# KleistLab/ADAPTed

Measured on AMD Instinct MI355X. Metric: reads/sec (adapter+polyA detect), RNA004 200k-sample reads, higher is better.
Workload: dtype f32 samples/statistics, f64 cumulative sums + LLR trace

## Files before the change

adapted_amd/csrc/adapted_hip.hip:

```cpp
#include <hip/hip_runtime.h>

#include <cmath>
#include <cstdio>
#include <cstring>
#include <cstdlib>
#include <string>
#include <vector>

#include "adapted_hip.h"
#include "handle.h"
#include "common.h"
__device__ unsigned long long g_dbg[ADP_NDBG] = {0};
__device__ unsigned long long g_bs_tally[ADP_NTALLY][8] = {{0}};
#include "llr_stream.h"
#include "n1_select.h"
#include "n1_fused.h"
#include "peaks.h"
#include "synth.h"
#include "validate.h"
#include "cand_stats2.h"
#include "series_pipe.h"
#include "cnn_topk.h"
#include "cnn_conv.h"
#include "cnn_conv_split.h"
// ... 449 lines not shown
                     const int32_t *tails = nullptr)
{
    hipStream_t st = h->stream;
    h->n1_fused_nmb = 0;
    MbState *mbs = h->mbs.as<MbState>();
    uint32_t *gh = h->ghist.as<uint32_t>(), *gb = h->gbelow.as<uint32_t>();
    unsigned long long *gc = h->gcnt.as<unsigned long long>();
    const int collect = ((long long)minibatch * T >= (1ll << 24)) ? 1 : 0;
    ALLOCCHK(collect && h->cbuf.ensure((size_t)n_mb * N1_CB_CAP * 4));
    uint32_t *cb = h->cbuf.as<uint32_t>();
    int bpm = 4096 / n_mb; if (bpm > 256) bpm = 256; if (bpm < 4) bpm = 4;
    dim3 hg(bpm, n_mb), pg(n_mb);
    const int pdiv = 32;
    int col_div = 1;
    if (T >= 8192) { col_div = T / (pdiv * 96); if (col_div > 64) col_div = 64; if (col_div < 2) col_div = 2; }
    int row_step = (col_div > 1) ? 1 : minibatch / 32; if (row_step < 1) row_step = 1;
    int sb = (minibatch + row_step - 1) / row_step; if (sb > bpm) sb = bpm; if (sb < 1) sb = 1;
    dim3 sg(sb, n_mb);
    const double thr = h->cfg.sig_norm_outlier_thresh;
    const long long fused_min = getenv("ADP_N1_FUSED_MIN") ? atoll(getenv("ADP_N1_FUSED_MIN")) : (1ll << 22);
    if ((long long)minibatch * T >= fused_min && T >= 64) {
        ALLOCCHK(h->cbuf.ensure((size_t)n_mb * N1_CB_CAP * 4) || h->fz.ensure((size_t)n_mb * sizeof(N1Fused)) ||
                 h->fcnt.ensure((size_t)n_mb * 8 * N1F_NCNT) || h->n1heavy.ensure((size_t)n_mb * N1H_WORDS * 4));
        cb = h->cbuf.as<uint32_t>();
        h->n1_fused_nmb = n_mb;
        N1Fused *fz = h->fz.as<N1Fused>();
        unsigned long long *fc = h->fcnt.as<unsigned long long>();
        HIPCHK(hipMemsetAsync(fc, 0, (size_t)n_mb * 8 * N1F_NCNT, st));
        uint32_t *hvy = h->n1heavy.as<uint32_t>();
        HIPCHK(hipMemsetAsync(hvy, 0, (size_t)n_mb * N1H_WORDS * 4, st));
        { Scope s(h, !profile ? nullptr : "k_n1 sample passes");
        const int s0 = (col_div > 1 && minibatch >= 64) ? env_int("ADP_N1_S0", 8) : 1;
        for (int mode = 0; mode < 2; mode++) {
            hipLaunchKernelGGL((k_n1_hist<0, SIG>), sg, dim3(N1_THREADS), 0, st, dsig, n, m, T, minibatch, mode, mbs, gh, gb, gc, row_step * (s0 > 1 ? s0 : 1), N1_ALWAYS, cb, 0, col_div, pdiv, tails);
            hipLaunchKernelGGL((k_n1_pick<0, N1_SAMPLE>), pg, dim3(256), 0, st, mbs, gh, gb, gc, mode, thr);
            hipLaunchKernelGGL((k_n1_hist<1, SIG>), sg, dim3(N1_THREADS), 0, st, dsig, n, m, T, minibatch, mode, mbs, gh, gb, gc, row_step, N1_ALWAYS, cb, 0, col_div, pdiv, tails);
            hipLaunchKernelGGL((k_n1_pick<1, N1_SAMPLE>), pg, dim3(256), 0, st, mbs, gh, gb, gc, mode, thr);
            hipLaunchKernelGGL(k_n1_fuse_setup, dim3((n_mb + 63) / 64), dim3(64), 0, st, mbs, fz, n_mb, mode);
        }
        hipLaunchKernelGGL(k_n1_heavy_scan<SIG>, dim3((sb + 3) / 4, n_mb), dim3(N1_THREADS), 0, st, dsig, n, m, T, minibatch, mbs, fz, hvy, row_step * 4, col_div, pdiv, tails);
        hipLaunchKernelGGL(k_n1_heavy_pick, pg, dim3(64), 0, st, mbs, fz, hvy, n_mb); }
        { Scope s(h, !profile ? nullptr : "k_n1_fused");
          hipLaunchKernelGGL(k_n1_fused<SIG>, hg, dim3(N1_THREADS), 0, st, dsig, n, m, T, minibatch, mbs, fz, fc, (float *)cb, hvy, tails); }
        { Scope s(h, !profile ? nullptr : "k_n1_fused_finish");
          hipLaunchKernelGGL(k_n1_fused_finish, pg, dim3(1024), 0, st, mbs, fz, fc, (const float *)cb, thr, (const uint32_t *)hvy); }
    }
    if ((long long)minibatch * T >= fused_min && T >= 64 && bpm < 128) hg = dim3(128, n_mb);
    for (int mode = 0; mode < 2; mode++) {
        hipLaunchKernelGGL((k_n1_hist<0, SIG>), sg, dim3(N1_THREADS), 0, st, dsig, n, m, T, minibatch, mode, mbs, gh, gb, gc, row_step, N1_ALWAYS, cb, 0, col_div, pdiv, tails);
        hipLaunchKernelGGL((k_n1_pick<0, N1_SAMPLE>), pg, dim3(256), 0, st, mbs, gh, gb, gc, mode, thr);
        hipLaunchKernelGGL((k_n1_hist<1, SIG>), sg, dim3(N1_THREADS), 0, st, dsig, n, m, T, minibatch, mode, mbs, gh, gb, gc, row_step, N1_ALWAYS, cb, 0, col_div, pdiv, tails);
        hipLaunchKernelGGL((k_n1_pick<1, N1_SAMPLE>), pg, dim3(256), 0, st, mbs, gh, gb, gc, mode, thr);
        { Scope s(h, !profile ? nullptr : (mode ? "k_n1_hist<1> mad" : "k_n1_hist<1> med"));
          hipLaunchKernelGGL((k_n1_hist<1, SIG>), hg, dim3(N1_THREADS), 0, st, dsig, n, m, T, minibatch, mode, mbs, gh, gb, gc, 1, N1_ALWAYS, cb, collect, 1, 8, tails); }
        hipLaunchKernelGGL((k_n1_pick<1, N1_FULL>), pg, dim3(256), 0, st, mbs, gh, gb, gc, mode, thr);
        hipLaunchKernelGGL(k_n1_finish, pg, dim3(1024), 0, st, mbs, cb, gc, gb, mode, thr);
        hipLaunchKernelGGL((k_n1_hist<0, SIG>), hg, dim3(N1_THREADS), 0, st, dsig, n, m, T, minibatch, mode, mbs, gh, gb, gc, 1, N1_IF_BAD, cb, 0, 1, 8, tails);
        hipLaunchKernelGGL((k_n1_pick<0, N1_FALLBACK>), pg, dim3(256), 0, st, mbs, gh, gb, gc, mode, thr);
        hipLaunchKernelGGL((k_n1_hist<1, SIG>), hg, dim3(N1_THREADS), 0, st, dsig, n, m, T, minibatch, mode, mbs, gh, gb, gc, 1, N1_IF_BAD, cb, 0, 1, 8, tails);
        hipLaunchKernelGGL((k_n1_pick<1, N1_FALLBACK>), pg, dim3(256), 0, st, mbs, gh, gb, gc, mode, thr);
        { Scope s(h, !profile ? nullptr : (mode ? "k_n1_hist<2> mad" : "k_n1_hist<2> med"));
          hipLaunchKernelGGL((k_n1_hist<2, SIG>), hg, dim3(N1_THREADS), 0, st, dsig, n, m, T, minibatch, mode, mbs, gh, gb, gc, 1, N1_IF_NOT_DONE, cb, 0, 1, 8, tails); }
        hipLaunchKernelGGL((k_n1_pick<2, N1_FULL>), pg, dim3(256), 0, st, mbs, gh, gb, gc, mode, thr);
    }
    return 0;
}

struct PhaseSync {
    hipEvent_t wait[3] = {nullptr, nullptr, nullptr};
    hipEvent_t done[3] = {nullptr, nullptr, nullptr};
};

static __device__ __host__ inline SigF32 sig_from(const SigF32 &s, size_t r0, int m) { return SigF32{s.base + r0 * (size_t)m}; }
static __device__ __host__ inline SigI16 sig_from(const SigI16 &s, size_t r0, int m) { return SigI16{s.base + r0 * (size_t)m, s.scale + r0, s.offset + r0, s.full_len + r0}; }
static inline SigIdx sig_subset(const SigF32 &s, const int32_t *sel) { return SigIdx{s.base, sel}; }
static inline SigIdxI16 sig_subset(const SigI16 &s, const int32_t *sel) { return SigIdxI16{s.base, s.scale, s.offset, s.full_len, sel}; }

static void launch_cumsum(adp_handle *h, int n)
{
    const int split = env_int("ADP_CUMSUM_GATHER", 1) != 0;
    hipLaunchKernelGGL(k_cumsum, dim3((n + 63) / 64), dim3(64), 0, h->stream, h->down.as<float>(), h->nvalid.as<int32_t>(), h->Lp, n,
                       h->nck, h->ck.as<double2>(), h->tail.as<double2>(), split);
    if (split)
        hipLaunchKernelGGL(k_cumsum_gather, dim3((n + 63) / 64), dim3(64), 0, h->stream, h->down.as<float>(), h->nvalid.as<int32_t>(), h->Lp, n,
                           h->nck, h->ck.as<double2>(), h->tail.as<double2>());
}

static int gains_tile_fast() { return env_int("ADP_GAINS_TILE_FAST", 1) != 0; }

#define G2_WINDOW_DEFAULT 1024
static int g2_window(int upto)
{
    const char *e = getenv("ADP_G2_WINDOW");
    if (!e || !*e) return upto >= 8 ? G2_WINDOW_DEFAULT : 0;
    const int w = env_int("ADP_G2_WINDOW", G2_WINDOW_DEFAULT);
    return w < 0 ? 0 : (w > (1 << 28) ? (1 << 28) : w);
}
static void launch_gains2(adp_handle *h, int n, int mbsize, double *pkv, int win, const int32_t *redo, const MbState *mbs = nullptr)
{
    hipLaunchKernelGGL(k_gains<2>, dim3((n + GAINS_WPB - 1) / GAINS_WPB), dim3(64 * GAINS_WPB), 0, h->stream, h->down.as<float>(), h->nvalid.as<int32_t>(), h->Lp, h->nck,
                       h->ck.as<double2>(), h->tail.as<double2>(), h->adapter_idx.as<int32_t>(), mbsize, mbs ? mbs : h->mbs.as<MbState>(),
                       h->trace.as<double>(), h->bmax.as<double>(), h->bmin.as<double>(), h->nsum, h->t1.as<int2>(), 0, h->pk.as<int32_t>(), h->npk.as<int32_t>(), h->Lp / 2 + 1, h->gstat.as<double>(), n, 5, pkv, gains_tile_fast(),
                       win, h->wend.as<int32_t>(), redo);
}

static void launch_polya_peak(adp_handle *h, int n, int mbsize, const double *pkv, bool windowed = false, bool redo_pass = false, const MbState *mbs = nullptr)
{
    const int grid = n < h->pslots ? n : h->pslots;
    hipLaunchKernelGGL(k_polya_peak, dim3(grid), dim3(64), (size_t)(((h->Lp / 2 + 1) + 8) / 16 + 2) * 4, h->stream, h->trace.as<double>(), h->nvalid.as<int32_t>(), h->Lp,
                       h->bmax.as<double>(), h->bmin.as<double>(), h->nsum, h->adapter_idx.as<int32_t>(), n, mbsize, mbs ? mbs : h->mbs.as<MbState>(),
                       h->pk.as<int32_t>(), h->mk.as<uint32_t>(), h->polya_idx.as<int32_t>(), h->npk.as<int32_t>(), pkv, env_int("ADP_PK_PREFIX", PK_PREFIX),
                       (windowed || redo_pass) ? h->wend.as<int32_t>() : (const int32_t *)nullptr, (windowed || redo_pass) ? h->redo.as<int32_t>() : (int32_t *)nullptr, redo_pass ? 1 : 0);
}

template <class SIG>
static int llr_enqueue(adp_handle *h, SIG dsig, const int32_t *dlen, int n, int m, int minibatch, int flags,
                       adp_row *rows_dev, int rows_kind , int32_t *mb_status_dev, double *mb_params_dev,
                       int upto, const PhaseSync *ps)
{
    int rc = 0;
    const int n_mb = (n + minibatch - 1) / minibatch;
    h->last_n = n; h->last_nmb = n_mb;
    ALLOCCHK(h->mbs.ensure((size_t)n_mb * sizeof(MbState)) || h->ghist.ensure((size_t)n_mb * N1_BINS * 4) || h->gbelow.ensure((size_t)n_mb * 8) || h->gcnt.ensure((size_t)n_mb * 8 * N1_NCNT));
    rc = alloc_all(h, n, true);
    if (rc) return rc;
    hipStream_t st = h->stream;
#ifdef ADP_ABLATE
    sync_ablate(h);
#endif
    if (ps && ps->wait[0]) HIPCHK(hipStreamWaitEvent(st, ps->wait[0], 0));
    MbState *mbs = h->mbs.as<MbState>();
    HIPCHK(hipMemsetAsync(mbs, 0, (size_t)n_mb * sizeof(MbState), st));
    HIPCHK(hipMemsetAsync(h->ghist.p, 0, (size_t)n_mb * N1_BINS * 4, st));
    HIPCHK(hipMemsetAsync(h->gbelow.p, 0, (size_t)n_mb * 8, st));
    HIPCHK(hipMemsetAsync(h->gcnt.p, 0, (size_t)n_mb * 8 * N1_NCNT, st));
    const int T = h->T;
    bool sp_forked = false, sp_done = false;
    if (h->L <= 0) {
        hipLaunchKernelGGL(k_mb_set_status, dim3((n_mb + 255) / 256), dim3(256), 0, st, mbs, n_mb, ADP_MB_EMPTY_TRACE);
        if (ps) for (int k = 0; k < 2; k++) { if (k && ps->wait[k]) HIPCHK(hipStreamWaitEvent(st, ps->wait[k], 0)); if (ps->done[k]) HIPCHK(hipEventRecord(ps->done[k], st)); }
    } else {
        const int32_t *tails = (flags & ADP_TAILS_NAN) ? dlen : nullptr;
        rc = launch_n1(h, dsig, n, m, T, minibatch, n_mb, true, tails);
        if (rc) return rc;
        const bool sp_fused = upto >= 8 && (flags & ADP_WITH_START_PEAK) && h->layout == ADP_LAYOUT_MINIBATCH &&
                              h->cfg.sp_downscale_factor == h->ds && h->off % h->ds == 0 && T > h->off && env_int("ADP_SP_FUSED", 1) != 0;
        if (sp_fused) {
            ALLOCCHK(h->sphead.ensure((size_t)n * sizeof(SpHead)));
            Scope s(h, "k_sp_head");
            hipLaunchKernelGGL(k_sp_head<SIG>, dim3(n), dim3(64), (size_t)64 * h->cfg.sp_downscale_factor * 4, st, dsig, dlen, n, m, h->cfg, h->off, h->sphead.as<SpHead>());
        }
        if (upto >= 2 && sp_fused) {
            { Scope s(h, "k_norm_pool");
              auto kern = (h->ds == 10 && std::is_same<SIG, SigF32>::value && env_int("ADP_NP_PREFETCH", 1)) ? k_norm_pool<SIG, true, 5> : k_norm_pool<SIG, true, 0>;
              hipLaunchKernelGGL(kern, dim3(n), dim3(256), (size_t)NP_TILE * h->ds * 4, st, dsig, m, T, h->off, h->ds, h->L, h->Lp,
                                 minibatch, mbs, h->down.as<float>(), h->nvalid.as<int32_t>(), (const int64_t *)nullptr,
                                 dlen, (flags & ADP_TAILS_NAN) ? 1 : 0, h->sphead.as<SpHead>(), (float)h->cfg.open_pore_pa); }
            const int cov0 = h->off / h->ds, cov1 = cov0 + (T - h->off) / h->ds;
            Scope s(h, "k_sp_tail");
            hipLaunchKernelGGL(k_sp_tail<SIG>, dim3(n), dim3(64), (size_t)64 * h->cfg.sp_downscale_factor * 4, st, dsig, dlen, n, m, h->cfg, cov0, cov1,
                               (const SpHead *)h->sphead.as<SpHead>(), h->sp.as<SpOut>());
            sp_done = true;
        } else if (upto >= 2) {
            Scope s(h, "k_norm_pool");
            const int64_t *rng = nullptr;
            if (h->layout == ADP_LAYOUT_SINGLE_READ) {
                ALLOCCHK(h->rng0.ensure((size_t)n * 16));
                std::vector<int64_t> hr((size_t)2 * n);
                for (int i = 0; i < n; i++) { hr[2 * i] = 0; hr[2 * i + 1] = T; }
                HIPCHK(hipMemcpyAsync(h->rng0.p, hr.data(), (size_t)n * 16, hipMemcpyHostToDevice, st));
                HIPCHK(hipStreamSynchronize(st));
                rng = h->rng0.as<int64_t>();
            }
            auto kern = (h->ds == 10 && !rng && std::is_same<SIG, SigF32>::value && env_int("ADP_NP_PREFETCH", 1)) ? k_norm_pool<SIG, false, 5> : k_norm_pool<SIG, false, 0>;
            hipLaunchKernelGGL(kern, dim3(n), dim3(256), (size_t)NP_TILE * h->ds * 4, st, dsig, m, T, h->off, h->ds, h->L, h->Lp,
                               minibatch, mbs, h->down.as<float>(), h->nvalid.as<int32_t>(), rng,
                               dlen, (flags & ADP_TAILS_NAN) ? 1 : 0, (SpHead *)nullptr, 0.f);
        }
        if (upto >= 2)
            hipLaunchKernelGGL(k_check_empty, dim3((n + 255) / 256), dim3(256), 0, st, h->nvalid.as<int32_t>(), n, minibatch, mbs);
        if (ps && ps->done[0]) HIPCHK(hipEventRecord(ps->done[0], st));
        if (upto >= 8 && (flags & ADP_WITH_START_PEAK) && !sp_fused) {
            HIPCHK(hipEventRecord(h->ev_fork, st));
            HIPCHK(hipStreamWaitEvent(h->stream2, h->ev_fork, 0));
            { Scope s(h, "k_start_peak", h->stream2);
              hipLaunchKernelGGL(k_start_peak<SIG>, dim3(n), dim3(64), (size_t)64 * h->cfg.sp_downscale_factor * 4, h->stream2, dsig, dlen, n, m, h->cfg, h->sp.as<SpOut>()); }
            HIPCHK(hipEventRecord(h->ev_join, h->stream2));
            sp_forked = true;
        }
        if (ps && ps->wait[1]) HIPCHK(hipStreamWaitEvent(st, ps->wait[1], 0));
        if (upto >= 3) {
            Scope s(h, "k_cumsum");
            launch_cumsum(h, n);
        }
        if (upto >= 4) {
            Scope s(h, "k_gains<1>");
            hipLaunchKernelGGL(k_gains<1>, dim3((n + GAINS_WPB - 1) / GAINS_WPB), dim3(64 * GAINS_WPB), 0, st, h->down.as<float>(), h->nvalid.as<int32_t>(), h->Lp, h->nck,
                               h->ck.as<double2>(), h->tail.as<double2>(), h->adapter_idx.as<int32_t>(), minibatch, mbs,
                               h->trace.as<double>(), h->bmax.as<double>(), h->bmin.as<double>(), h->nsum, h->t1.as<int2>(), 0, h->pk.as<int32_t>(), h->npk.as<int32_t>(), h->Lp / 2 + 1, h->gstat.as<double>(), n, h->oh1, nullptr, gains_tile_fast());
        }
        if (upto >= 5) {
            Scope s(h, "k_adapter_peak");
            hipLaunchKernelGGL(k_adapter_peak, dim3(n), dim3(64), 0, st, h->trace.as<double>(), h->nvalid.as<int32_t>(), h->Lp,
                               h->bmax.as<double>(), h->bmin.as<double>(), h->nsum, h->t1.as<int2>(), minibatch, mbs,
                               h->cfg.adapter_peak_prominence, h->cfg.adapter_peak_rel_height,
                               h->cfg.adapter_peak_width / h->ds, h->adapter_idx.as<int32_t>(), h->gstat.as<double>());
        }
        double *pkvp = (env_int("ADP_PK_VALUES", 1) && h->pkv.cap >= (size_t)n * (h->Lp / 2 + 1) * 8) ? h->pkv.as<double>() : nullptr;
        int win = g2_window(upto);
        if (win > 0 && (win + 1 + TRACE_TILE - 1) / TRACE_TILE * TRACE_TILE >= h->L) win = 0;
        if (upto >= 6) {
            if (win > 0) HIPCHK(hipMemsetAsync(h->redo.p, 0, 4, st));
            Scope s(h, "k_gains<2>");
            launch_gains2(h, n, minibatch, pkvp, win, nullptr);
        }
        if (upto >= 7) {
            { Scope s(h, "k_polya_peak");
              launch_polya_peak(h, n, minibatch, pkvp, win > 0); }
            if (win > 0) {
                { Scope s(h, "k_gains<2> redo");
                  launch_gains2(h, n, minibatch, pkvp, 0, h->redo.as<int32_t>()); }
                { Scope s(h, "k_polya_peak redo");
                  launch_polya_peak(h, n, minibatch, pkvp, false, true); }
            }
        }
        if (ps && ps->done[1]) HIPCHK(hipEventRecord(ps->done[1], st));
    }
    if (upto >= 8) {
        if (ps && ps->wait[2]) HIPCHK(hipStreamWaitEvent(st, ps->wait[2], 0));
        if (h->L > 0)
            hipLaunchKernelGGL(k_llr_bounds, dim3((n + 255) / 256), dim3(256), 0, st, h->adapter_idx.as<int32_t>(),
                               h->polya_idx.as<int32_t>(), n, h->ds, h->pos_off, h->bounds.as<int64_t>(), h->topk_none.as<int8_t>(), h->layout == ADP_LAYOUT_SINGLE_READ ? 1 : 0);
        rc = launch_validate(h, dsig, dlen, n, m, 1, minibatch, true);
        if (rc) return rc;
        if (flags & ADP_WITH_START_PEAK) {
            if (sp_forked) HIPCHK(hipStreamWaitEvent(st, h->ev_join, 0));
            else if (!sp_done) {
                Scope s(h, "k_start_peak");
                hipLaunchKernelGGL(k_start_peak<SIG>, dim3(n), dim3(64), (size_t)64 * h->cfg.sp_downscale_factor * 4, st, dsig, dlen, n, m, h->cfg, h->sp.as<SpOut>());
            }
            hipLaunchKernelGGL(k_sp_decorate, dim3((n + 255) / 256), dim3(256), 0, st, h->sp.as<SpOut>(), h->rows.as<adp_row>(), n, 0,
                               (const int32_t *)nullptr);
        }
        if (rows_dev)
            HIPCHK(hipMemcpyAsync(rows_dev, h->rows.p, (size_t)n * sizeof(adp_row), (hipMemcpyKind)rows_kind, st));
    }
    if (mb_status_dev)
        hipLaunchKernelGGL(k_mb_status_out, dim3((n_mb + 255) / 256), dim3(256), 0, st, mbs, n_mb, mb_status_dev);
    if (mb_params_dev)
        hipLaunchKernelGGL(k_mb_params_out, dim3((n_mb + 255) / 256), dim3(256), 0, st, mbs, n_mb, mb_params_dev);
    if (ps && ps->done[2]) HIPCHK(hipEventRecord(ps->done[2], st));
    HIPCHK(hipGetLastError());
    return ADP_OK;
}

static bool trunc_wanted(int flags, const adp_row *rows) { return (flags & ADP_FLAG_TRUNCATED) && rows; }
static int trunc_supported(const adp_handle *h)
{
    const adp_cfg &c = h->cfg;
    const int W = c.median_shift_window;
    if (!c.mvs_detect_check) { g_err = "ADP_FLAG_TRUNCATED needs mvs_detect_check (its tests are the MVS check's)"; return ADP_ERR_UNSUPPORTED; }
    if (c.mvs_detect_overwrite) { g_err = "ADP_FLAG_TRUNCATED does not go with mvs_detect_overwrite"; return ADP_ERR_UNSUPPORTED; }
    if (h->layout == ADP_LAYOUT_SINGLE_READ) { g_err = "ADP_FLAG_TRUNCATED does not go with the single-read layout"; return ADP_ERR_UNSUPPORTED; }
    if (W > PT_WMAX) { g_err = "ADP_FLAG_TRUNCATED: median_shift_window is longer than the tail test holds in LDS (4096)"; return ADP_ERR_UNSUPPORTED; }
    if (c.pA_var_window < 1 || c.pA_mean_window < 1 || c.pA_var_window + 2 >= W || c.pA_mean_window + 2 >= W) {
        g_err = "ADP_FLAG_TRUNCATED: pA_mean_window and pA_var_window must lie in [1, median_shift_window - 3]"; return ADP_ERR_UNSUPPORTED;
    }
    return 0;
}
static int trunc_enqueue_t1(adp_handle *h, const float *dsig, const int32_t *dlen, int n, int m, adp_row *rows)
{
    int8_t *verdict;
    ALLOCCHK(h->pt_sel.ensure((size_t)n * 4));
    RCCHK(sub_carve(h, [&](Carve &c) { verdict = c.take<int8_t>(n); }));
    unsigned int *counts = phase_counts(h, OPW_PT);
    h->pt_looked = true;
    HIPCHK(hipMemsetAsync(counts, 0, 12, h->stream));
    { Scope s(h, "k_pt_t1");
      hipLaunchKernelGGL(k_pt_t1, dim3(n), dim3(64), (size_t)3 * h->cfg.median_shift_window * 4, h->stream, dsig, dlen, n, m, h->cfg, rows, verdict); }
    { Scope s(h, "k_pt_select");
      hipLaunchKernelGGL(k_pt_select, dim3(1), dim3(SEL_THREADS), 0, h->stream, (const int8_t *)verdict, n, h->pt_sel.as<int32_t>(),
                         h->op_used.as<unsigned int>() + 4, counts); }
    return 0;
}
static int trunc_run_t2(adp_handle *h, const float *dsig, const int32_t *dlen, int m, adp_row *rows, int n_t1)
{
    int rc = alloc_all(h, n_t1, false);
    if (rc) return rc;
    const size_t N = (size_t)n_t1;
    int64_t *b2; int32_t *dlen_sub; int8_t *tsub; adp_row *rows2;
    RCCHK(sub_carve(h, [&](Carve &c) {
        b2 = c.take<int64_t>(2 * N); dlen_sub = c.take<int32_t>(N); tsub = c.take<int8_t>(N); rows2 = c.take<adp_row>(N);
    }));
    const int32_t *sel = h->pt_sel.as<int32_t>();
    { Scope s(h, "k_pt_gather");
      hipLaunchKernelGGL(k_pt_gather, dim3((n_t1 + 255) / 256), dim3(256), 0, h->stream, sel, n_t1, m, dlen, (const adp_row *)rows, dlen_sub, b2, tsub); }
    const ValBufs vb{b2, tsub, rows2};
    rc = launch_validate(h, SigIdx{dsig, sel}, dlen_sub, n_t1, m, 1, n_t1, false, &vb, true);
    if (rc) return rc;
    { Scope s(h, "k_pt_merge");
      hipLaunchKernelGGL(k_pt_merge, dim3(n_t1), dim3(64), 0, h->stream, sel, n_t1, (const adp_row *)rows2, rows, phase_counts(h, OPW_PT)); }
    HIPCHK(hipGetLastError());
    return 0;
}
static int trunc_finish(adp_handle *h, const float *dsig, const int32_t *dlen, int n, int m, adp_row *rows)
{
    unsigned int n_pt = 0;
    RCCHK(trunc_enqueue_t1(h, dsig, dlen, n, m, rows));
    const int rc = arena_end(h, false, nullptr, nullptr, &n_pt);
    if (rc || !n_pt) return rc;
    RCCHK(trunc_run_t2(h, dsig, dlen, m, rows, (int)n_pt));
    HIPCHK(hipStreamSynchronize(h->stream));
    return arena_end(h);
}
static bool reseg_wanted(int flags, const adp_row *rows) { return (flags & ADP_LLR_RESEGMENT) && rows; }
static int reseg_supported(const adp_handle *h, int flags)
{
    if (flags & ADP_FLAG_TRUNCATED) { g_err = "ADP_LLR_RESEGMENT does not go with ADP_FLAG_TRUNCATED (the truncation look validates from start 0)"; return ADP_ERR_UNSUPPORTED; }
    if (h->cfg.mvs_detect_overwrite) { g_err = "ADP_LLR_RESEGMENT does not go with mvs_detect_overwrite"; return ADP_ERR_UNSUPPORTED; }
    if (h->layout == ADP_LAYOUT_SINGLE_READ) { g_err = "ADP_LLR_RESEGMENT does not go with the single-read layout"; return ADP_ERR_UNSUPPORTED; }
    return 0;
}
struct RsPieces {
    Piece<int64_t> b2, starts; Piece<int32_t> dlen_sub; Piece<int8_t> tsub; Piece<MbState> mbs_sub; Piece<adp_row> rows2;
    void take(Carve &c, size_t N)
    {
        b2 = c.take<int64_t>(2 * N); starts = c.take<int64_t>(N); dlen_sub = c.take<int32_t>(N); tsub = c.take<int8_t>(N);
// ... 1525 lines not shown
```

adapted_amd/csrc/llr_stream.h:

```cpp
#pragma once
#include <type_traits>
#include "common.h"
#include "log_cr.h"
#include "wave_stats.h"

extern __device__ unsigned long long g_dbg[ADP_NDBG];

#define NP_TILE 512
struct SpHead {
    int32_t valid, max_idx, a2, e0;
    float mx;
    int32_t op_end;
    int32_t op_head, op_body, hit;
    int32_t pad;
};

template <class SIG, bool SP = false, int NQ = 0>
__global__ void __launch_bounds__(256) k_norm_pool(SIG sig, int m, int T, int off, int ds, int L, int Lp,
                                                   int mbsize, const MbState *__restrict__ mbs,
                                                   float *__restrict__ down, int32_t *__restrict__ nvalid,
                                                   const int64_t *__restrict__ ranges, const int32_t *__restrict__ full_len,
                                                   int tails_nan = 0, SpHead *__restrict__ sp_head = nullptr, float sp_thr = 0.f)
{
    extern __shared__ __attribute__((aligned(16))) float tile[];
    __shared__ int s_nan;
    __shared__ __attribute__((aligned(16))) int s_sp[2];
    const int r = blockIdx.x;
    const MbState st = mbs[r / mbsize];
    if (st.status != ADP_MB_OK) { if (threadIdx.x == 0) nvalid[r] = 0; return; }
    const float med = st.med, mad = st.mad, lo = st.lo, hi = st.hi;
    int Lseg = T - off;
    if (ranges) {
        long long a = ranges[2 * r], b = ranges[2 * r + 1];
        long long lim = full_len[r] < T ? full_len[r] : T;
        if (b > lim) b = lim;
        off = (int)a;
        Lseg = (int)(b > a ? b - a : 0);
        L = (Lseg + ds - 1) / ds;
        if (L > Lp) L = Lp;
    }
    const typename SIG::Row row = sig.row(r, m) + off;
    if (threadIdx.x == 0) s_nan = 0;
    int my_nan = 0;
    float sp_mx = 0.f;
    int sp_a2 = 0, sp_e0 = 0, sp_op_end = 0, sp_hit = 0x7fffffff, sp_op = 0x7fffffff;
    const int sp_full = (T - off) / ds;
    const int sp_pb0 = off / ds;
    if (SP) {
        const SpHead hd = sp_head[r];
        sp_mx = hd.mx; sp_a2 = hd.valid ? hd.a2 : 0; sp_e0 = hd.valid ? hd.e0 : 0; sp_op_end = hd.op_end;
        if (threadIdx.x < 2) s_sp[threadIdx.x] = 0x7fffffff;
    }
    int L_ok = L;
    if (tails_nan && !ranges) {
        long long lv = (long long)full_len[r] - off;
        if (lv < Lseg) { if (lv < 0) lv = 0; L_ok = (int)(lv / ds); }
    }
    const int tile_n = NP_TILE * ds;
    const bool vec = row.vec_ok() && ((tile_n & 3) == 0);
    const bool fast_div = fdiv_ok(mad);
    const float rmad = 1.0f / mad;
    auto norm1 = [&](float c) {
        c = c < lo ? lo : c;
        c = c > hi ? hi : c;
        return fast_div ? fdiv_shared(c - med, mad, rmad) : (c - med) / mad;
    };
    const bool use_pf = NQ > 0 && vec && tile_n / 4 == NQ * 256;
    float4 pre[NQ > 0 ? NQ : 1];
    auto fetch = [&](int tb_) {
        const int base_ = tb_ * ds;
        const typename SIG::Row rowb = row + base_;
#pragma unroll
        for (int u = 0; u < (NQ > 0 ? NQ : 1); u++) {
            const int q = threadIdx.x + u * 256;
            const int idx = base_ + 4 * q;
            float4 v = make_float4(0.f, 0.f, 0.f, 0.f);
            if (idx + 3 < Lseg) v = rowb.f4s(q);
            else {
                if (idx < Lseg) v.x = row[idx];
                if (idx + 1 < Lseg) v.y = row[idx + 1];
                if (idx + 2 < Lseg) v.z = row[idx + 2];
            }
            pre[u] = v;
        }
    };
    if (use_pf && L_ok > 0 && L > 0) fetch(0);
    for (int tb = 0; tb < L; tb += NP_TILE) {
        const int base = tb * ds;
        if (tb >= L_ok) {
            for (int jj = threadIdx.x; jj < NP_TILE; jj += 256) if (tb + jj < L) { down[(size_t)r * Lp + tb + jj] = __builtin_nanf(""); my_nan++; }
            continue;
        }
        __syncthreads();
        if (use_pf) {
#pragma unroll
            for (int u = 0; u < (NQ > 0 ? NQ : 1); u++) {
                const int q = threadIdx.x + u * 256;
                const int idx = base + 4 * q;
                float4 v = pre[u];
                if (!SP) {
                    v.x = idx < Lseg ? norm1(v.x) : 0.f; v.y = idx + 1 < Lseg ? norm1(v.y) : 0.f;
                    v.z = idx + 2 < Lseg ? norm1(v.z) : 0.f; v.w = idx + 3 < Lseg ? norm1(v.w) : 0.f;
                }
                reinterpret_cast<float4 *>(tile)[q] = v;
            }
        } else if (vec) {
            const typename SIG::Row rowb = row + base;
            for (int q = threadIdx.x; q < tile_n / 4; q += 256) {
                const int idx = base + 4 * q;
                float4 v = make_float4(0.f, 0.f, 0.f, 0.f);
                if (SP) {
                    const float padv = -__builtin_inff();
                    v = make_float4(padv, padv, padv, padv);
                    if (idx + 3 < Lseg) v = rowb.f4s(q);
                    else {
                        if (idx < Lseg) v.x = row[idx];
                        if (idx + 1 < Lseg) v.y = row[idx + 1];
                        if (idx + 2 < Lseg) v.z = row[idx + 2];
                    }
                } else if (idx + 3 < Lseg) { v = rowb.f4s(q); v.x = norm1(v.x); v.y = norm1(v.y); v.z = norm1(v.z); v.w = norm1(v.w); }
                else {
                    if (idx < Lseg) v.x = norm1(row[idx]);
                    if (idx + 1 < Lseg) v.y = norm1(row[idx + 1]);
                    if (idx + 2 < Lseg) v.z = norm1(row[idx + 2]);
                }
                reinterpret_cast<float4 *>(tile)[q] = v;
            }
        } else {
            for (int i = threadIdx.x; i < tile_n; i += 256) {
                int idx = base + i;
                if (SP) tile[i] = (idx < Lseg) ? row[idx] : -__builtin_inff();
                else tile[i] = (idx < Lseg) ? norm1(row[idx]) : 0.0f;
            }
        }
        __syncthreads();
        if (use_pf) { const int nx = tb + NP_TILE; if (nx < L && nx < L_ok) fetch(nx); }
        for (int jj = threadIdx.x; jj < NP_TILE; jj += 256) {
            const int j = tb + jj;
            if (j < L) {
                const float *p = tile + jj * ds;
                float s;
                if (SP) {
                    const int nin = Lseg - j * ds;
                    if (nin >= ds) s = pw_leaf_f32(ds, [&](int k) { return norm1(p[k]); });
                    else s = pw_leaf_f32(ds, [&](int k) { return k < nin ? norm1(p[k]) : 0.0f; });
                    if (j < sp_full) {
                        const int g = sp_pb0 + j;
                        if (g >= sp_a2 && g < sp_e0) {
                            const float v = pw_leaf_f32(ds, [&](int k) { return p[k]; }) / (float)ds;
                            if (v > sp_mx && g < sp_hit) sp_hit = g;
                        }
                        const int i0 = off + j * ds;
                        if (i0 < sp_op_end && sp_op == 0x7fffffff) {
                            for (int k = 0; k < ds; k++) if (i0 + k < sp_op_end && p[k] > sp_thr) { sp_op = i0 + k; break; }
                        }
                    }
                } else s = pw_leaf_f32(ds, [&](int k) { return p[k]; });
                float pooled = s / (float)ds;
                down[(size_t)r * Lp + j] = pooled;
                if (pooled != pooled) my_nan++;
            }
        }
    }
    if (SP) {
        sp_hit = wave_min(sp_hit); sp_op = wave_min(sp_op);
        if (lane_id() == 0) { if (sp_hit != 0x7fffffff) atomicMin(&s_sp[0], sp_hit); if (sp_op != 0x7fffffff) atomicMin(&s_sp[1], sp_op); }
    }
    my_nan = wave_sum(my_nan);
    if (lane_id() == 0 && my_nan) atomicAdd(&s_nan, my_nan);
    __syncthreads();
    if (threadIdx.x == 0) {
        nvalid[r] = L - s_nan;
        if (SP) { sp_head[r].hit = s_sp[0]; sp_head[r].op_body = s_sp[1]; }
    }
}

static __device__ __forceinline__ bool csum_uniform(int n) { return wave_max(n) - wave_min(n) < 8 * CK; }
__global__ void __launch_bounds__(64) k_cumsum(const float *__restrict__ down, const int32_t *__restrict__ nvalid, int Lp, int n_reads,
                                               int nck, double2 *__restrict__ ck, double2 *__restrict__ tail, int split)
{
    const int r = blockIdx.x * 64 + threadIdx.x;
    const int n = r < n_reads ? nvalid[r] : 0;
    if (split && csum_uniform(n)) return;
    if (r >= n_reads) return;
    const float *s = down + (size_t)r * Lp;
    double2 *c = ck + (size_t)r * nck;
    double a = 0.0, b = 0.0;
    double2 t = make_double2(0.0, 0.0);
    const float4 *s4 = reinterpret_cast<const float4 *>(s);
    auto block = [&](int j0, const float4 (&q)[4]) {
        c[j0 / CK] = make_double2(a, b);
        const float v[16] = {q[0].x, q[0].y, q[0].z, q[0].w, q[1].x, q[1].y, q[1].z, q[1].w, q[2].x, q[2].y, q[2].z, q[2].w, q[3].x, q[3].y, q[3].z, q[3].w};
        if (j0 + CK < n) {
#pragma unroll
            for (int u = 0; u < CK; u++) { const double x = (double)v[u]; a += x; b += x * x; }
        } else {
#pragma unroll
            for (int u = 0; u < CK; u++) {
                const int j = j0 + u;
                if (j < n) {
                    if (j == n - 1) t = make_double2(a, b);
                    double x = (double)v[u];
                    a += x;
                    b += x * x;
                }
            }
        }
    };
    constexpr int PFL = 2;
    float4 q[PFL][2][4];
    const int last_line = Lp / (2 * CK) - 1;
    auto ldl = [&](int line, float4 (&qq)[2][4]) {
        const float4 *p4 = s4 + (line < last_line ? line : last_line) * (2 * CK / 4);
#pragma unroll
        for (int e = 0; e < 8; e++) qq[e >> 2][e & 3] = p4[e];
    };
#pragma unroll
    for (int d = 0; d < PFL; d++) ldl(d, q[d]);
    for (int j0 = 0; j0 < n; j0 += PFL * 2 * CK) {
        const int line = j0 / (2 * CK);
#pragma unroll
        for (int d = 0; d < PFL; d++) {
            const int j1 = j0 + d * 2 * CK;
            if (d == 0 || j1 < n) block(j1, q[d][0]);
            if (j1 + CK < n) block(j1 + CK, q[d][1]);
            ldl(line + PFL + d, q[d]);
        }
    }
    tail[r] = t;
}

#define CSUM_Q 8
typedef double csum_d2 __attribute__((ext_vector_type(2)));
__global__ void __launch_bounds__(64) k_cumsum_gather(const float *__restrict__ down, const int32_t *__restrict__ nvalid, int Lp, int n_reads,
                                                      int nck, double2 *__restrict__ ck, double2 *__restrict__ tail)
{
    __shared__ __attribute__((aligned(16))) csum_d2 cks_[64 * (CSUM_Q + 1)];
    LDS csum_d2 *cks = (LDS csum_d2 *)cks_;
    const int ln = threadIdx.x, r0 = blockIdx.x * 64;
    const int r = r0 + ln;
    const int n = r < n_reads ? nvalid[r] : 0;
    if (!csum_uniform(n)) return;
    const int nmax = wave_max(n);
    const float *s = down + (size_t)(r < n_reads ? r : n_reads - 1) * Lp;
    double a = 0.0, b = 0.0;
    double2 t = make_double2(0.0, 0.0);
    const float4 *s4 = reinterpret_cast<const float4 *>(s);
    auto block = [&](int j0, int slot, const float4 (&q)[4]) {
        cks[ln * (CSUM_Q + 1) + slot] = (csum_d2){a, b};
        const float v[16] = {q[0].x, q[0].y, q[0].z, q[0].w, q[1].x, q[1].y, q[1].z, q[1].w, q[2].x, q[2].y, q[2].z, q[2].w, q[3].x, q[3].y, q[3].z, q[3].w};
        if (j0 + CK < n) {
#pragma unroll
            for (int u = 0; u < CK; u++) { const double x = (double)v[u]; a += x; b += x * x; }
        } else {
#pragma unroll
            for (int u = 0; u < CK; u++) {
                const int j = j0 + u;
                if (j < n) {
                    if (j == n - 1) t = make_double2(a, b);
                    double x = (double)v[u];
                    a += x;
                    b += x * x;
                }
            }
        }
    };
    static_assert(CSUM_Q % 4 == 0, "a group is a whole number of prefetch rounds of two lines");
    constexpr int PFL = 2, LPG = CSUM_Q / 2;
    float4 q[PFL][2][4];
    const int last_line = n > 0 ? (n - 1) / (2 * CK) : 0;
    auto ldl = [&](int line, float4 (&qq)[2][4]) {
        const float4 *p4 = s4 + (line < last_line ? line : last_line) * (2 * CK / 4);
#pragma unroll
        for (int e = 0; e < 8; e++) qq[e >> 2][e & 3] = p4[e];
    };
#pragma unroll
    for (int d = 0; d < PFL; d++) ldl(d, q[d]);
    for (int g0 = 0; g0 * (CSUM_Q * CK) < nmax; g0++) {
#pragma unroll
        for (int l2 = 0; l2 < LPG; l2 += PFL) {
#pragma unroll
            for (int d = 0; d < PFL; d++) {
                const int line = g0 * LPG + l2 + d, j1 = line * 2 * CK, slot = 2 * (l2 + d);
                if (j1 < n) block(j1, slot, q[d][0]);
                if (j1 + CK < n) block(j1 + CK, slot + 1, q[d][1]);
                ldl(line + PFL, q[d]);
            }
        }
        ws_sync();
// ... 358 lines not shown
```

Baseline: 1.195 million.

## Double-buffer half tiles in norm_pool with register prefetch two stages ahead

```diff
diff --git a/adapted_amd/csrc/adapted_hip.hip b/adapted_amd/csrc/adapted_hip.hip
--- a/adapted_amd/csrc/adapted_hip.hip
+++ b/adapted_amd/csrc/adapted_hip.hip
@@ -625,7 +625,7 @@
         }
         if (upto >= 2 && sp_fused) {
             { Scope s(h, "k_norm_pool");
-              auto kern = (h->ds == 10 && std::is_same<SIG, SigF32>::value && env_int("ADP_NP_PREFETCH", 1)) ? k_norm_pool<SIG, true, 5> : k_norm_pool<SIG, true, 0>;
+              auto kern = (h->ds == NP_PIPE_DS && env_int("ADP_NP_PREFETCH", 1)) ? k_norm_pool<SIG, true, std::is_same<SIG, SigF32>::value> : k_norm_pool<SIG, true, false>;
               hipLaunchKernelGGL(kern, dim3(n), dim3(256), (size_t)NP_TILE * h->ds * 4, st, dsig, m, T, h->off, h->ds, h->L, h->Lp,
                                  minibatch, mbs, h->down.as<float>(), h->nvalid.as<int32_t>(), (const int64_t *)nullptr,
                                  dlen, (flags & ADP_TAILS_NAN) ? 1 : 0, h->sphead.as<SpHead>(), (float)h->cfg.open_pore_pa); }
@@ -645,7 +645,7 @@
                 HIPCHK(hipStreamSynchronize(st));
                 rng = h->rng0.as<int64_t>();
             }
-            auto kern = (h->ds == 10 && !rng && std::is_same<SIG, SigF32>::value && env_int("ADP_NP_PREFETCH", 1)) ? k_norm_pool<SIG, false, 5> : k_norm_pool<SIG, false, 0>;
+            auto kern = (h->ds == NP_PIPE_DS && !rng && env_int("ADP_NP_PREFETCH", 1)) ? k_norm_pool<SIG, false, std::is_same<SIG, SigF32>::value> : k_norm_pool<SIG, false, false>;
             hipLaunchKernelGGL(kern, dim3(n), dim3(256), (size_t)NP_TILE * h->ds * 4, st, dsig, m, T, h->off, h->ds, h->L, h->Lp,
                                minibatch, mbs, h->down.as<float>(), h->nvalid.as<int32_t>(), rng,
                                dlen, (flags & ADP_TAILS_NAN) ? 1 : 0, (SpHead *)nullptr, 0.f);
diff --git a/adapted_amd/csrc/llr_stream.h b/adapted_amd/csrc/llr_stream.h
--- a/adapted_amd/csrc/llr_stream.h
+++ b/adapted_amd/csrc/llr_stream.h
@@ -15,7 +15,10 @@
     int32_t pad;
 };
 
-template <class SIG, bool SP = false, int NQ = 0>
+#define NP_HALF (NP_TILE / 2)
+#define NP_PIPE_DS 10
+typedef float adp_v2f __attribute__((ext_vector_type(2)));
+template <class SIG, bool SP = false, bool PIPE = false>
 __global__ void __launch_bounds__(256) k_norm_pool(SIG sig, int m, int T, int off, int ds, int L, int Lp,
                                                    int mbsize, const MbState *__restrict__ mbs,
                                                    float *__restrict__ down, int32_t *__restrict__ nvalid,
@@ -60,51 +63,102 @@
     const bool vec = row.vec_ok() && ((tile_n & 3) == 0);
     const bool fast_div = fdiv_ok(mad);
     const float rmad = 1.0f / mad;
-    auto norm1 = [&](float c) {
+    auto norm_as = [&](float c, bool fast) {
         c = c < lo ? lo : c;
         c = c > hi ? hi : c;
-        return fast_div ? fdiv_shared(c - med, mad, rmad) : (c - med) / mad;
+        return fast ? fdiv_shared(c - med, mad, rmad) : (c - med) / mad;
     };
-    const bool use_pf = NQ > 0 && vec && tile_n / 4 == NQ * 256;
-    float4 pre[NQ > 0 ? NQ : 1];
-    auto fetch = [&](int tb_) {
-        const int base_ = tb_ * ds;
-        const typename SIG::Row rowb = row + base_;
-#pragma unroll
-        for (int u = 0; u < (NQ > 0 ? NQ : 1); u++) {
-            const int q = threadIdx.x + u * 256;
-            const int idx = base_ + 4 * q;
-            float4 v = make_float4(0.f, 0.f, 0.f, 0.f);
-            if (idx + 3 < Lseg) v = rowb.f4s(q);
-            else {
-                if (idx < Lseg) v.x = row[idx];
-                if (idx + 1 < Lseg) v.y = row[idx + 1];
-                if (idx + 2 < Lseg) v.z = row[idx + 2];
-            }
-            pre[u] = v;
-        }
+    auto norm1 = [&](float c) { return norm_as(c, fast_div); };
+    bool piped = false;
+    auto pipeline = [&](auto fast_c) {
+        auto norm1 = [&](float c) { return norm_as(c, decltype(fast_c)::value); };
+        piped = true;
+        constexpr int DS = NP_PIPE_DS, HS = NP_HALF * DS, NL = HS / 512;
+        static_assert(HS % 512 == 0 && NP_HALF == 256, "a thread pools one value and carries NL whole 8-byte loads per half tile");
+        const int live = L < L_ok ? L : L_ok;
+        const int H = (live + NP_HALF - 1) / NP_HALF;
+        const GLB adp_v2f *row2 = reinterpret_cast<const GLB adp_v2f *>(row.p);
+        adp_v2f pre[NL];
+        auto fetch = [&](int h_) {
+            const int q0 = h_ * (HS / 2) + threadIdx.x;
+            if ((h_ + 1) * HS <= Lseg) {
+#pragma unroll
+                for (int u = 0; u < NL; u++) pre[u] = __builtin_nontemporal_load(row2 + q0 + u * 256);
+            } else {
+#pragma unroll
+                for (int u = 0; u < NL; u++) {
+                    const int idx = 2 * (q0 + u * 256);
+                    adp_v2f v = {0.f, 0.f};
+                    if (idx + 1 < Lseg) v = __builtin_nontemporal_load(row2 + q0 + u * 256);
+                    else if (idx < Lseg) v.x = row[idx];
+                    pre[u] = v;
+                }
+            }
+        };
+        auto stage = [&](int h_) {
+            LDS adp_v2f *dst = (LDS adp_v2f *)(tile + (h_ & 1) * HS) + threadIdx.x;
+            if (SP) {
+#pragma unroll
+                for (int u = 0; u < NL; u++) dst[u * 256] = pre[u];
+            } else if ((h_ + 1) * HS <= Lseg) {
+#pragma unroll
+                for (int u = 0; u < NL; u++) { adp_v2f v = pre[u]; v.x = norm1(v.x); v.y = norm1(v.y); dst[u * 256] = v; }
+            } else {
+#pragma unroll
+                for (int u = 0; u < NL; u++) {
+                    const int idx = 2 * (h_ * (HS / 2) + threadIdx.x + u * 256);
+                    adp_v2f v = pre[u];
+                    v.x = idx < Lseg ? norm1(v.x) : 0.f; v.y = idx + 1 < Lseg ? norm1(v.y) : 0.f;
+                    dst[u * 256] = v;
+                }
+            }
+        };
+        if (H > 0) { fetch(0); stage(0); }
+        if (H > 1) fetch(1);
+        __syncthreads();
+        for (int h = 0; h < H; h++) {
+            if (h + 1 < H) stage(h + 1);
+            if (h + 2 < H) fetch(h + 2);
+            const int j = h * NP_HALF + threadIdx.x;
+            if (j < L) {
+                const float *p = tile + (h & 1) * HS + threadIdx.x * DS;
+                float s;
+                if (SP) {
+                    const int nin = Lseg - j * DS;
+                    if (nin >= DS) s = pw_leaf_f32(DS, [&](int k) { return norm1(p[k]); });
+                    else s = pw_leaf_f32(DS, [&](int k) { return k < nin ? norm1(p[k]) : 0.0f; });
+                    if (j < sp_full) {
+                        const int g = sp_pb0 + j;
+                        if (g >= sp_a2 && g < sp_e0) {
+                            const float v = pw_leaf_f32(DS, [&](int k) { return p[k]; }) / (float)DS;
+                            if (v > sp_mx && g < sp_hit) sp_hit = g;
+                        }
+                        const int i0 = off + j * DS;
+                        if (i0 < sp_op_end && sp_op == 0x7fffffff) {
+                            for (int k = 0; k < DS; k++) if (i0 + k < sp_op_end && p[k] > sp_thr) { sp_op = i0 + k; break; }
+                        }
+                    }
+                } else s = pw_leaf_f32(DS, [&](int k) { return p[k]; });
+                float pooled = s / (float)DS;
+                down[(size_t)r * Lp + j] = pooled;
+                if (pooled != pooled) my_nan++;
+            }
+            __syncthreads();
+        }
+        for (int j = H * NP_HALF + threadIdx.x; j < L; j += NP_HALF) { down[(size_t)r * Lp + j] = __builtin_nanf(""); my_nan++; }
     };
-    if (use_pf && L_ok > 0 && L > 0) fetch(0);
-    for (int tb = 0; tb < L; tb += NP_TILE) {
+    if constexpr (PIPE) if (row.vec_ok() && ds == NP_PIPE_DS && !ranges) {
+        if (fast_div) pipeline(std::true_type{}); else pipeline(std::false_type{});
+    }
+    if (PIPE && !piped && threadIdx.x == 0) atomicAdd(&g_dbg[61], 1ull);
+    for (int tb = 0; tb < L && !piped; tb += NP_TILE) {
         const int base = tb * ds;
         if (tb >= L_ok) {
             for (int jj = threadIdx.x; jj < NP_TILE; jj += 256) if (tb + jj < L) { down[(size_t)r * Lp + tb + jj] = __builtin_nanf(""); my_nan++; }
             continue;
         }
         __syncthreads();
-        if (use_pf) {
-#pragma unroll
-            for (int u = 0; u < (NQ > 0 ? NQ : 1); u++) {
-                const int q = threadIdx.x + u * 256;
-                const int idx = base + 4 * q;
-                float4 v = pre[u];
-                if (!SP) {
-                    v.x = idx < Lseg ? norm1(v.x) : 0.f; v.y = idx + 1 < Lseg ? norm1(v.y) : 0.f;
-                    v.z = idx + 2 < Lseg ? norm1(v.z) : 0.f; v.w = idx + 3 < Lseg ? norm1(v.w) : 0.f;
-                }
-                reinterpret_cast<float4 *>(tile)[q] = v;
-            }
-        } else if (vec) {
+        if (vec) {
             const typename SIG::Row rowb = row + base;
             for (int q = threadIdx.x; q < tile_n / 4; q += 256) {
                 const int idx = base + 4 * q;
@@ -134,7 +188,6 @@
             }
         }
         __syncthreads();
-        if (use_pf) { const int nx = tb + NP_TILE; if (nx < L && nx < L_ok) fetch(nx); }
         for (int jj = threadIdx.x; jj < NP_TILE; jj += 256) {
             const int j = tb + jj;
             if (j < L) {
```

Measured after the change: 1.177 million. -1.5%, worse.
